# LuckyLYM/Zebra

Hardware: AMD Instinct MI355X
Metric: temporal edges/sec embedded (k=20, 2-layer) (higher is better)
Workload: dtype f64+f32

## Files before the change

### zebra_amd/csrc/aggregate.hip

```cpp
#include "common.hpp"
#include "embed_out_body.hpp"
#include "fc1_tile.hpp"

using namespace zt;
using namespace zt::dense;

namespace {

constexpr int MAX_MT = 5;
constexpr int MAX_MT_BIG = 16;
constexpr int MAX_MT_BIG_WIDE = 8;

#ifdef ZT_AGG_STAMP
__device__ unsigned long long g_agg[8];
#define AGG_STAMP(i) do { if (threadIdx.x == 0) { const long long t__ = clock64(); atomicAdd(&g_agg[i], (unsigned long long)(t__ - t_prev__)); t_prev__ = t__; } } while (0)
#else
#define AGG_STAMP(i) do { } while (0)
#endif

template <bool TAB, int MMT = MAX_MT, int NW = NTW>
__global__ __launch_bounds__(AGG_THREADS) void k_fc1_agg(FcAggArgs a, int rq, int mt_count, int lda)
{
    extern __shared__ __attribute__((aligned(16))) char smem[];
    const float *__restrict__ memory = a.memory, *__restrict__ efeat = a.efeat, *__restrict__ overlay = a.overlay;
// ... 232 lines not shown
        g_nb[tid] = nb; g_ei[tid] = ei; g_dt[tid] = d; wn[tid] = wv;
    }
    const int cc = tid & 127;
    const float wc = cc < T ? time_w[cc] : 0.f;
    const int col0 = wave * 16 + r16;
    const float bias0 = col0 < D ? b1[col0] : 0.f, bias1 = (wave < 3 && col0 + 64 < D) ? b1[col0 + 64] : 0.f;
    __syncthreads();
    AGG_STAMP(0);

    f32x4 acc[5][2];
#pragma unroll
    for (int a = 0; a < 5; ++a) {
        const int nb4[4] = {g_nb[a * 16 + g4 * 4 + 0], g_nb[a * 16 + g4 * 4 + 1], g_nb[a * 16 + g4 * 4 + 2], g_nb[a * 16 + g4 * 4 + 3]};
#pragma unroll
        for (int j = 0; j < 4; ++j) {
            const float *pr = P + (size_t)nb4[j] * DP + col0;
            acc[a][0][j] = pr[0];
            acc[a][1][j] = pr[wave < 3 ? 64 : 0];
        }
    }
    if (tid < ROWS) {
        const int q = tid / KK;
        float my_sum = 0.f;
#pragma unroll
        for (int j = 0; j < KK; ++j) my_sum += wn[q * KK + j];
        wnn[tid] = (my_sum == 0.f) ? 0.f : wn[tid] / my_sum;
        if (tid < rows && tid - q * KK == 0) S[(size_t)m * N + q0 + q] = (my_sum == 0.f) ? 0.f : 1.f;
    }
    AGG_STAMP(1);
    if (F == 1) {
        if (tid < ROWS) A[(size_t)tid * lda] = ef1;
    } else if (F > 0) {
        constexpr int GU = 8;
        const bool vecF = (F & 3) == 0 && ((size_t)efeat & 15) == 0;
        if (vecF) {
            const int F4 = F >> 2;
            const unsigned mF4 = fastdiv_magic((unsigned)F4);
            for (int f0 = tid; f0 < ROWS * F4; f0 += AGG_THREADS * GU) {
                f32x4 v[GU];
#pragma unroll
                for (int u = 0; u < GU; ++u) {
                    const int f = f0 + u * AGG_THREADS;
                    const int g = fastdiv(f, mF4), c = f - g * F4;
                    v[u] = (f < ROWS * F4 && g < rows) ? *reinterpret_cast<const f32x4 *>(efeat + (size_t)g_ei[g] * F + 4 * c)
                                                      : f32x4{0.f, 0.f, 0.f, 0.f};
                }
#pragma unroll
                for (int u = 0; u < GU; ++u) {
                    const int f = f0 + u * AGG_THREADS;
                    const int g = fastdiv(f, mF4), c = f - g * F4;
                    if (f < ROWS * F4) *reinterpret_cast<f32x4 *>(A + (size_t)g * lda + 4 * c) = v[u];
                }
            }
        } else {
            const unsigned mF = fastdiv_magic((unsigned)F);
            for (int f0 = tid; f0 < ROWS * F; f0 += AGG_THREADS * GU) {
                float v[GU];
#pragma unroll
                for (int u = 0; u < GU; ++u) {
                    const int f = f0 + u * AGG_THREADS;
                    const int g = fastdiv(f, mF), c = f - g * F;
                    v[u] = (f < ROWS * F && g < rows) ? efeat[(size_t)g_ei[g] * F + c] : 0.f;
                }
#pragma unroll
                for (int u = 0; u < GU; ++u) {
                    const int f = f0 + u * AGG_THREADS;
                    const int g = fastdiv(f, mF), c = f - g * F;
                    if (f < ROWS * F) A[(size_t)g * lda + c] = v[u];
                }
            }
        }
    }
    {
        const int g0 = (tid >> 7) * 40;
        const bool is_cos = cc < T;
        if (is_cos || F + cc < K1p) {
            float *dst = A + (size_t)g0 * lda + F + cc;
            float xmax = 0.f;
#pragma unroll 2
            for (int i = 0; i < 40; i += 4) {
                const f32x4 d4 = *reinterpret_cast<const f32x4 *>(g_dt + g0 + i);
#pragma unroll
                for (int u = 0; u < 4; ++u) {
                    const float x = d4[u] * wc;
                    xmax = fmaxf(xmax, fabsf(x));
                    dst[(size_t)(i + u) * lda] = time_cosf_fast(x);
                }
            }
            if (!is_cos) {
                for (int i = 0; i < 40; ++i) dst[(size_t)i * lda] = 0.f;
            } else if (!(xmax < 4.0e6f)) {
                for (int i = 0; i < 40; ++i) dst[(size_t)i * lda] = time_cosf(g_dt[g0 + i] * wc);
            }
        }
    }
    AGG_STAMP(2);
    AGG_STAMP(3);
    __syncthreads();
    AGG_STAMP(4);

    {
        const float *bp = W1p + (size_t)col0 * K1p + 4 * g4;
        const int K4 = (F + T + 3) & ~3, nchunk = K4 >> 4, nrem = (K4 & 15) >> 2;
        if (wave < 3) d100_mfma<2>(A, lda, bp, K1p, nchunk, nrem, r16, g4, acc);
        else          d100_mfma<1>(A, lda, bp, K1p, nchunk, nrem, r16, g4, acc);
    }
    AGG_STAMP(5);
    __syncthreads();

    float *Hs = A;
    {
        float *hp = Hs + (size_t)(g4 * 4) * LDH + col0;
#pragma unroll
        for (int a = 0; a < 5; ++a) {
            const f32x4 w4 = *reinterpret_cast<const f32x4 *>(wnn + a * 16 + g4 * 4);
#pragma unroll
            for (int j = 0; j < 4; ++j) {
                float v = acc[a][0][j] + bias0;
                v = v > 0.f ? v : 0.f;
                hp[(size_t)(a * 16 + j) * LDH] = v * w4[j];
            }
        }
        if (wave < 3) {
#pragma unroll
            for (int a = 0; a < 5; ++a) {
                const f32x4 w4 = *reinterpret_cast<const f32x4 *>(wnn + a * 16 + g4 * 4);
#pragma unroll
                for (int j = 0; j < 4; ++j) {
                    float v1 = acc[a][1][j] + bias1;
                    v1 = v1 > 0.f ? v1 : 0.f;
                    hp[(size_t)(a * 16 + j) * LDH + 64] = v1 * w4[j];
                }
            }
        }
    }
    __syncthreads();
    AGG_STAMP(6);
    if (cc < D) {
        for (int q = tid >> 7; q < nq; q += 2) {
            const float *hq = Hs + (size_t)(q * KK) * LDH + cc;
            float s = 0.f;
#pragma unroll
            for (int j = 0; j < KK; ++j) s += hq[(size_t)j * LDH];
            H[((size_t)m * N + q0 + q) * D + cc] = s;
        }
    }
    AGG_STAMP(7);
}

#ifdef ZT_DIAG
__device__ unsigned long long g_regclk[4 * 1024];
#endif
constexpr int REG_NS = 26;
constexpr int REG_NB = 7;
constexpr int REG_FRAG_GROUPS = (REG_NB * REG_NS + 3) / 4;

__global__ void k_pack_reg_frag(const float *__restrict__ W1t, int K2p, float *__restrict__ image)
{
    const int i = blockIdx.x * blockDim.x + threadIdx.x;
    if (i >= REG_FRAG_GROUPS * 64 * 4) return;
    const int e = i & 3, lane = (i >> 2) & 63, G = i >> 8;
    const int q = 4 * G + e, b = q / REG_NS, st = q % REG_NS;
    image[i] = q < REG_NB * REG_NS ? W1t[(16 * b + (lane & 15)) * K2p + 4 * st + (lane >> 4)] : 0.f;
}

template <int KK, int DBG = 0>
__global__ __launch_bounds__(AGG_THREADS, 1) void k_fc1_agg_reg(
    const float *__restrict__ P, const float *__restrict__ efeat, const float *__restrict__ time_w, long long num_nodes,
    long long num_edges, int F, long long N, int M, const int *__restrict__ nbr, const int *__restrict__ eix,
    const float *__restrict__ dt, const float *__restrict__ w, const float *__restrict__ Wfrag,
    const float *__restrict__ b1, float *__restrict__ H, float *__restrict__ S, int *status,
    const int *gate_word, int gate_target, int *gate_latch)
{
    constexpr int D = 100, T = 100, DP = 112, ROWS = 80, RQ = ROWS / KK;
    static_assert(KK % 4 == 0 && ROWS % KK == 0, "groups of 4 rows must not straddle query rows");
    __shared__ int s_nb[AGG_WAVES][ROWS];
    __shared__ __attribute__((aligned(16))) float s_dt[AGG_WAVES][ROWS];
    __shared__ __attribute__((aligned(16))) float s_w[AGG_WAVES][ROWS];
    __shared__ float s_sum[AGG_WAVES][4];
    __shared__ __attribute__((aligned(16))) float s_ef[AGG_WAVES][ROWS * 4];
    const int lane = threadIdx.x & 63, wave = threadIdx.x >> 6;
    const int r16 = lane & 15, g4 = lane >> 4;
    int *nb_s = s_nb[wave];
    float *dt_s = s_dt[wave], *w_s = s_w[wave], *sum_s = s_sum[wave], *ef_s = s_ef[wave];
#ifdef ZT_DIAG
    const unsigned long long wall_in = DBG ? __builtin_amdgcn_s_memrealtime() : 0ull;
#endif

    float Breg[REG_NB][REG_NS];
    {
        const f32x4 *Wf = reinterpret_cast<const f32x4 *>(Wfrag) + lane;
        static_assert(REG_FRAG_GROUPS % 2 == 0, "two batches");
        constexpr int HB = REG_FRAG_GROUPS / 2;
#pragma unroll
        for (int half = 0; half < 2; ++half) {
            f32x4 v[HB];
#pragma unroll
            for (int i = 0; i < HB; ++i) v[i] = Wf[(half * HB + i) * 64];
            __builtin_amdgcn_sched_barrier(0);
#pragma unroll
            for (int i = 0; i < HB; ++i)
#pragma unroll
                for (int e = 0; e < 4; ++e) {
                    const int q = 4 * (half * HB + i) + e;
                    if (q < REG_NB * REG_NS) asm volatile("v_accvgpr_write_b32 %0, %1" : "=a"(Breg[q / REG_NS][q % REG_NS]) : "v"(v[i][e]));
                }
            __builtin_amdgcn_sched_barrier(0);
        }
    }
    float freq[REG_NS];
#pragma unroll
    for (int st = 0; st < REG_NS; ++st) {
        const int kc = 4 * st + g4 - F;
        freq[st] = (kc >= 0 && kc < T) ? time_w[kc] : 0.f;
    }
    float bias[REG_NB];
#pragma unroll
    for (int b = 0; b < REG_NB; ++b) bias[b] = (16 * b + r16) < D ? b1[16 * b + r16] : 0.f;

#ifdef ZT_DIAG
    const unsigned long long clk0 = DBG ? __builtin_amdgcn_s_memtime() : 0ull, wall0 = DBG ? __builtin_amdgcn_s_memrealtime() : 0ull;
#endif
    const long long tpm = (N + RQ - 1) / RQ;
    const long long n_tiles = tpm * M;
    const long long stride = (long long)gridDim.x * AGG_WAVES;
    long long tile = (long long)blockIdx.x * AGG_WAVES + wave;

    int pf_nb[2] = {0, 0}, pf_ei[2] = {0, 0};
    float pf_dt[2] = {0.f, 0.f}, pf_w[2] = {0.f, 0.f};
    auto fetch = [&](long long t) {
        const long long m = t / tpm, q0 = (t - m * tpm) * RQ;
        const int rows = (int)((N - q0) < RQ ? (N - q0) : RQ) * KK;
        const size_t mb = ((size_t)m * N + q0) * KK;
#pragma unroll
        for (int h = 0; h < 2; ++h) {
            const int row = h * 64 + lane;
            const bool in = row < rows && (h == 0 || lane < ROWS - 64);
            pf_nb[h] = in ? nbr[mb + row] : 0;
            pf_ei[h] = in ? eix[mb + row] : 0;
            pf_dt[h] = in ? dt[mb + row] : 0.f;
            pf_w[h] = in ? w[mb + row] : 0.f;
        }
    };
    float pf_ef[2][4] = {{0.f, 0.f, 0.f, 0.f}, {0.f, 0.f, 0.f, 0.f}};
    auto fetch_ef = [&]() {
#pragma unroll
        for (int h = 0; h < 2; ++h) {
            const int ei = pf_ei[h];
            const bool ok = ei >= 0 && ei < num_edges && (h == 0 || lane < ROWS - 64);
#pragma unroll
            for (int c = 0; c < 4; ++c) pf_ef[h][c] = (ok && c < F) ? efeat[(size_t)ei * F + c] : 0.f;
        }
    };
    member_gate_enter(gate_word, gate_target, status, gate_latch);
    if (tile < n_tiles) { fetch(tile); fetch_ef(); }

#pragma nounroll
    for (; tile < n_tiles; tile += stride) {
        const long long m = tile / tpm, q0 = (tile - m * tpm) * RQ;
        const int nq = (int)((N - q0) < RQ ? (N - q0) : RQ);
#pragma unroll
        for (int h = 0; h < 2; ++h) {
            const int row = h * 64 + lane;
            if (h == 0 || lane < ROWS - 64) {
                int nb = pf_nb[h], ei = pf_ei[h];
                if (nb < 0 || nb >= num_nodes || ei < 0 || ei >= num_edges) { atomicExch(status, ZT_ERR_RANGE); nb = 0; ei = 0; }
                nb_s[row] = nb; dt_s[row] = pf_dt[h]; w_s[row] = pf_w[h];
                *reinterpret_cast<f32x4 *>(ef_s + 4 * row) = f32x4{pf_ef[h][0], pf_ef[h][1], pf_ef[h][2], pf_ef[h][3]};
            }
        }
        wave_sync();
        if (lane < RQ) {
            f32x4 wv[KK / 4];
#pragma unroll
            for (int j = 0; j < KK / 4; ++j) wv[j] = *reinterpret_cast<const f32x4 *>(w_s + lane * KK + 4 * j);
            float sm = 0.f;
#pragma unroll
            for (int j = 0; j < KK; ++j) sm += wv[j / 4][j % 4];
            sum_s[lane] = sm;
            if (lane < nq) S[(size_t)m * N + q0 + lane] = (sm == 0.f) ? 0.f : 1.f;
        }
        wave_sync();
#pragma unroll
        for (int h = 0; h < 2; ++h) {
            const int row = h * 64 + lane;
            if (h == 0 || lane < ROWS - 64) {
                const float qs = sum_s[row / KK];
                w_s[row] = (qs == 0.f) ? 0.f : pf_w[h] / qs;
            }
        }
        wave_sync();
        const bool has_next = tile + stride < n_tiles;
        if (has_next) fetch(tile + stride);

        float Hloc[RQ][REG_NB];
#pragma unroll
        for (int q = 0; q < RQ; ++q)
#pragma unroll
            for (int b = 0; b < REG_NB; ++b) Hloc[q][b] = 0.f;

        f32x4 acc[REG_NB];
        float accv[REG_NB][4], Pv[2][REG_NB][4], wn_cur[4], wn_prv[4];
        auto load_P = [&](int x) {
            const int4 nb4 = *reinterpret_cast<const int4 *>(nb_s + x * 16 + 4 * g4);
            const float *p0 = P + (size_t)nb4.x * DP + r16, *p1 = P + (size_t)nb4.y * DP + r16,
                        *p2 = P + (size_t)nb4.z * DP + r16, *p3 = P + (size_t)nb4.w * DP + r16;
#pragma unroll
            for (int b = 0; b < REG_NB; ++b) {
                Pv[x & 1][b][0] = p0[16 * b]; Pv[x & 1][b][1] = p1[16 * b]; Pv[x & 1][b][2] = p2[16 * b]; Pv[x & 1][b][3] = p3[16 * b];
            }
        };
        if (!(DBG & 4)) { load_P(0); load_P(1); }
#pragma unroll
        for (int a = 0; a <= 5; ++a) {
            float dta = 0.f, A_next[2] = {0.f, 0.f};
            if (a > 0) {
#pragma unroll
                for (int b = 0; b < REG_NB; ++b)
#pragma unroll
                    for (int j = 0; j < 4; ++j) accv[b][j] = acc[b][j];
#pragma unroll
                for (int j = 0; j < 4; ++j) wn_prv[j] = wn_cur[j];
            }
            if (a < 5) {
                dta = dt_s[a * 16 + r16];
                const float ef = ef_s[4 * (a * 16 + r16) + (g4 & 3)];
                const f32x4 w4 = *reinterpret_cast<const f32x4 *>(w_s + a * 16 + 4 * g4);
#pragma unroll
                for (int j = 0; j < 4; ++j) wn_cur[j] = w4[j];
#pragma unroll
                for (int b = 0; b < REG_NB; ++b) acc[b] = f32x4{bias[b], bias[b], bias[b], bias[b]};
                A_next[0] = (DBG & 1) ? dta * freq[0] : time_cosf_rev(dta * freq[0]);
                A_next[1] = (DBG & 1) ? dta * freq[1] : time_cosf_rev(dta * freq[1]);
                if (g4 < F) A_next[0] = ef;
                if (a == 2 && has_next) fetch_ef();
            }
            __builtin_amdgcn_sched_barrier(0);
            const int ap = a > 0 ? a - 1 : 0;
            const int q_lo = (16 * ap) / KK, q_hi = (16 * ap + 15) / KK;
#pragma unroll
            for (int st0 = 0; st0 < REG_NS; st0 += 2) {
                if (a == 5 && st0 >= REG_NB) break;
                const float A_cur[2] = {A_next[0], A_next[1]};
                if (a < 5) {
#pragma unroll
                    for (int u = 0; u < 2; ++u)
                        if (st0 + 2 + u < REG_NS)
                            A_next[u] = (DBG & 1) ? dta * freq[st0 + 2 + u] : time_cosf_rev(dta * freq[st0 + 2 + u]);
#pragma unroll
                    for (int u = 0; u < 2; ++u)
#pragma unroll
                        for (int b = 0; b < REG_NB; ++b)
                            acc[b] = __builtin_amdgcn_mfma_f32_16x16x4f32(A_cur[u], Breg[b][st0 + u], acc[b], 0, 0, 0);
                }
#pragma unroll
                for (int u = 0; u < 2; ++u) {
                    const int st = st0 + u;
                    if (!(a > 0 && st < REG_NB)) continue;
                    const int b = st;
                    float part = 0.f;
#pragma unroll
                    for (int j = 0; j < 4; ++j) {
                        float v = accv[b][j] + ((DBG & 2) ? 0.f : Pv[ap & 1][b][j]);
                        v = v > 0.f ? v : 0.f;
                        part += (DBG & 2) ? v : v * wn_prv[j];
                    }
                    if (DBG & 2) {
                        Hloc[q_lo][b] += part;
                    } else {
                        const int pi = __float_as_int(part);
                        const auto h = __builtin_amdgcn_permlane32_swap(pi, pi, false, false);
                        const auto lo = __builtin_amdgcn_permlane16_swap(h[0], h[0], false, false);
                        const auto hi = __builtin_amdgcn_permlane16_swap(h[1], h[1], false, false);
                        const float pg[4] = {__int_as_float(lo[0]), __int_as_float(lo[1]), __int_as_float(hi[0]), __int_as_float(hi[1])};
#pragma unroll
                        for (int g = 0; g < 4; ++g) {
                            const int q = (16 * ap + 4 * g) / KK;
                            if (q < RQ) Hloc[q][b] += pg[g];
                        }
                    }
                    asm volatile("" : "+v"(Hloc[q_lo][b]));
                    if (q_hi != q_lo && q_hi < RQ) asm volatile("" : "+v"(Hloc[q_hi][b]));
                }
                if (a >= 1 && a <= 3 && st0 == REG_NB + 1 && !(DBG & 4)) load_P(a + 1);
                __builtin_amdgcn_sched_barrier(0);
            }
        }
#pragma unroll
        for (int q = 0; q < RQ; ++q) {
            if (g4 == (q & 3) && q < nq) {
                float *hrow = H + ((size_t)m * N + q0 + q) * D;
#pragma unroll
                for (int b = 0; b < REG_NB; ++b)
                    if (16 * b + r16 < D) hrow[16 * b + r16] = Hloc[q][b];
            }
        }
        wave_sync();
    }
#ifdef ZT_DIAG
    if (DBG && lane == 0 && blockIdx.x * AGG_WAVES + wave < 1024) {
        unsigned long long *o = g_regclk + 4 * (blockIdx.x * AGG_WAVES + wave);
        o[0] = __builtin_amdgcn_s_memtime() - clk0; o[1] = wall0; o[2] = __builtin_amdgcn_s_memrealtime();
        o[3] = wall_in;
    }
#endif
}


constexpr int EO3_NT = 7, EO3_KC = 7, EO3_DP = 112, EO3_LDY = 116;
constexpr int EO3_FRAG = EO3_NT * EO3_KC * 256;

__device__ __forceinline__ void eo3_fill(float *Wl, const float *__restrict__ Wp, int tid)
{
    constexpr int PER = (EO3_NT * EO3_KC * 64 + 255) / 256;
    f32x4 v[PER];
#pragma unroll
    for (int q = 0; q < PER; ++q) {
        const int idx = tid + q * 256, frag = idx >> 6, ln = idx & 63;
        const int b = frag / EO3_KC, c = frag - b * EO3_KC;
        v[q] = idx < EO3_NT * EO3_KC * 64
                   ? *reinterpret_cast<const f32x4 *>(Wp + (size_t)(16 * b + (ln & 15)) * EO3_DP + 16 * c + 4 * (ln >> 4))
                   : f32x4{0.f, 0.f, 0.f, 0.f};
    }
#pragma unroll
    for (int q = 0; q < PER; ++q) {
        const int idx = tid + q * 256;
        if (idx < EO3_NT * EO3_KC * 64) reinterpret_cast<f32x4 *>(Wl)[idx] = v[q];
    }
}

template <int HG>
__global__ __launch_bounds__(AGG_THREADS, 1) void k_embed_out3(
    const float *__restrict__ memory, long long num_nodes, const int *__restrict__ nodes, long long N, int D, int M,
    const float *__restrict__ H, const float *__restrict__ S, const float *__restrict__ fc2_p,
    const float *__restrict__ fc2_b, const float *__restrict__ fc1s_p, const float *__restrict__ fc1s_b,
    const float *__restrict__ fc2s_p, const float *__restrict__ fc2s_b, float *__restrict__ out, int *status, int n_src)
{
    extern __shared__ __attribute__((aligned(16))) char smem[];
    float *W0 = reinterpret_cast<float *>(smem);
    const int tid = threadIdx.x, lane = tid & 63, wave = tid >> 6, r16 = lane & 15, g4 = lane >> 4;
    const int OW = D * (M + 1);
    const long long tiles = (N + 15) / 16;
    const f32x4 zero4 = {0.f, 0.f, 0.f, 0.f};
    bool cin[EO3_KC];
#pragma unroll
    for (int c = 0; c < EO3_KC; ++c) cin[c] = 16 * c + 4 * g4 < D;
    const f32x4 *Wf0 = reinterpret_cast<const f32x4 *>(W0) + lane;

    if ((int)blockIdx.x < n_src) {
        float *W1 = W0 + EO3_FRAG;
        float *Y = W1 + EO3_FRAG + wave * 16 * EO3_LDY;
        eo3_fill(W0, fc1s_p, tid);
        eo3_fill(W1, fc2s_p, tid);
        float b1v[EO3_NT], b2v[EO3_NT];
#pragma unroll
        for (int b = 0; b < EO3_NT; ++b) {
            b1v[b] = 16 * b + r16 < D ? fc1s_b[16 * b + r16] : 0.f;
            b2v[b] = 16 * b + r16 < D ? fc2s_b[16 * b + r16] : 0.f;
        }
        const f32x4 *Wf1 = reinterpret_cast<const f32x4 *>(W1) + lane;
        const long long stride = (long long)n_src * AGG_WAVES;
        long long t = (long long)blockIdx.x * AGG_WAVES + wave;
        auto node_of = [&](long long tt) -> int { return (tt < tiles && tt * 16 + r16 < N) ? nodes[tt * 16 + r16] : -1; };
        auto rows_of = [&](int nd, f32x4 (&a)[EO3_KC]) {
            const bool ok = nd >= 0 && nd < num_nodes;
#pragma unroll
            for (int c = 0; c < EO3_KC; ++c)
                a[c] = (ok && cin[c]) ? *reinterpret_cast<const f32x4 *>(memory + (size_t)nd * D + 16 * c + 4 * g4) : zero4;
        };
        int nd_cur = node_of(t), nd_nxt = node_of(t + stride);
        f32x4 a[EO3_KC], an[EO3_KC];
        if (t < tiles) rows_of(nd_cur, a);
        __syncthreads();
        for (; t < tiles; t += stride) {
            const long long r0 = t * 16;
            if (r0 + r16 < N && (nd_cur < 0 || nd_cur >= num_nodes)) atomicExch(status, ZT_ERR_RANGE);
            rows_of(nd_nxt, an);
            nd_cur = nd_nxt;
            nd_nxt = node_of(t + 2 * stride);
            f32x4 acc1[EO3_NT];
#pragma unroll
            for (int b = 0; b < EO3_NT; ++b) acc1[b] = zero4;
#pragma unroll
            for (int c = 0; c < EO3_KC; ++c) {
                f32x4 w[EO3_NT];
#pragma unroll
                for (int b = 0; b < EO3_NT; ++b) w[b] = Wf0[(b * EO3_KC + c) * 64];
#pragma unroll
                for (int j = 0; j < 4; ++j)
#pragma unroll
                    for (int b = 0; b < EO3_NT; ++b) acc1[b] = __builtin_amdgcn_mfma_f32_16x16x4f32(a[c][j], w[b][j], acc1[b], 0, 0, 0);
            }
#pragma unroll
            for (int b = 0; b < EO3_NT; ++b)
#pragma unroll
                for (int j = 0; j < 4; ++j) {
                    const float v = acc1[b][j] + b1v[b];
                    Y[(4 * g4 + j) * EO3_LDY + 16 * b + r16] = (16 * b + r16 < D && v > 0.f) ? v : 0.f;
                }
            wave_sync();
            f32x4 acc[EO3_NT];
#pragma unroll
            for (int b = 0; b < EO3_NT; ++b) acc[b] = zero4;
#pragma unroll
            for (int c = 0; c < EO3_KC; ++c) {
                const f32x4 y = *reinterpret_cast<const f32x4 *>(Y + r16 * EO3_LDY + 16 * c + 4 * g4);
                f32x4 w[EO3_NT];
#pragma unroll
                for (int b = 0; b < EO3_NT; ++b) w[b] = Wf1[(b * EO3_KC + c) * 64];
#pragma unroll
                for (int j = 0; j < 4; ++j)
#pragma unroll
                    for (int b = 0; b < EO3_NT; ++b) acc[b] = __builtin_amdgcn_mfma_f32_16x16x4f32(y[j], w[b][j], acc[b], 0, 0, 0);
            }
#pragma unroll
            for (int b = 0; b < EO3_NT; ++b) {
// ... 128 lines not shown
    size_t lds2;
    size_t off_w1p, off_H, off_S, off_fc2t, off_fc1st, off_fc2st, off_w1t, off_wm, off_wl, off_wfrag, total;
    int hg;
};

bool tile_shape(int Kp, int Dp, int k, int T, int *lda_out, int *mt_out, int *rq_out, size_t *lds_out, int max_mt = MAX_MT)
{
    const int lda = Kp + 4;
    int mt = max_mt;
    while (mt > 1 && ((size_t)mt * 16 * lda * 4 + (size_t)mt * 16 * 16) > (size_t)AGG_LDS_BUDGET) --mt;
    int rq = (mt * 16) / k;
    if (rq < 1) {
        mt = (k + 15) / 16;
        rq = 1;
        if (mt > max_mt || ((size_t)mt * 16 * lda * 4 + (size_t)mt * 16 * 16) > (size_t)AGG_LDS_BUDGET) return false;
    }
    mt = (rq * k + 15) / 16;
    if ((size_t)mt * 16 * (Dp + 1) * 4 > (size_t)mt * 16 * lda * 4) return false;
    *lda_out = lda; *mt_out = mt; *rq_out = rq;
    *lds_out = (size_t)mt * 16 * lda * 4 + (size_t)mt * 16 * 16 + (size_t)T * 4;
    return true;
}

bool split_fits(int D, int F, int T, int k) { return k <= ZT_MAX_K_WIDE && fc1_agg_split_rows(D, F, T) > 0; }

bool make_plan(int64_t N, int D, int F, int T, int M, int k, EmbedPlan &p)
{
    if (!width_supported(D)) return false;
    const int K1 = D + F + T;
    p.Dp = round_up(D, 16);
    p.K1p = round_up(K1, 16);
    const bool big = k > MAX_MT * 16;
    const int max_mt = big ? (p.Dp > 16 * NTW * AGG_WAVES ? MAX_MT_BIG_WIDE : MAX_MT_BIG) : MAX_MT;
    const bool full_ok = tile_shape(p.K1p, p.Dp, k, T, &p.lda, &p.mt, &p.rq, &p.lds, max_mt);
    if (!full_ok) { p.mt = 0; p.rq = 1; p.lda = p.K1p + 4; p.lds = 0; }
    p.K2p = round_up(F + T, 16);
    p.mt2 = 0;
    if (!(full_ok || big) || !tile_shape(p.K2p, p.Dp, k, T, &p.lda2, &p.mt2, &p.rq2, &p.lds2, max_mt)) p.mt2 = 0;
    if (p.mt == 0 && p.mt2 == 0 && !split_fits(D, F, T, k)) return false;
    size_t o = 0;
    auto take = [&](size_t bytes) { size_t r = o; o += (bytes + 255) & ~(size_t)255; return r; };
    p.off_w1p = take((size_t)p.Dp * p.K1p * 4);
    p.off_fc2t = take((size_t)p.Dp * p.Dp * 4);
    p.off_fc1st = take((size_t)p.Dp * p.Dp * 4);
    p.off_fc2st = take((size_t)p.Dp * p.Dp * 4);
    p.off_w1t = take((size_t)p.Dp * p.K2p * 4);
    p.off_wm = take((size_t)p.Dp * p.Dp * 4);
    p.hg = fc1_agg_wide_supported(D, F, T, k) ? k / 4 : 1;
    p.off_wl = take(p.hg > 1 ? fc1_agg_wide_weight_bytes() : 0);
    p.off_wfrag = take((size_t)REG_FRAG_GROUPS * 64 * 4 * 4);
    p.off_H = take((size_t)M * N * D * 4 * p.hg);
    p.off_S = take((size_t)M * N * 4);
    p.total = o;
    return true;
}

KernelPlan plan_kernels(int64_t N, int D, int F, int T, int M, int k, bool have_table, bool training, int agg_choice,
                        int out_choice, EmbedPlan &p)
{
    KernelPlan kp{AggKernel::unsupported, OutForm::tiled, Refusal::shape, 0, 0, 0, 0, 1};
    static_assert(16 * NTW * AGG_WAVES == 128 && 16 * NTW_WIDE * AGG_WAVES == MAX_D, "the N-tiles cover D <= 128 / D <= 256");
    if (!make_plan(N, D, F, T, M, k, p)) return kp;
    const bool big = k > MAX_MT * 16;
    const bool tab = have_table && !training && p.mt2 > 0;
    const bool special = tab && agg_choice != ZT_AGG_GENERIC;
    if (training ? (big || p.mt == 0) : (!tab && p.mt == 0)) {
        if (!split_fits(D, F, T, k)) { kp.refusal = Refusal::no_split; return kp; }
        kp.agg = AggKernel::split;
    } else if (special && p.hg > 1) {
        kp.agg = AggKernel::wide;
    } else if (special && D == 100 && T == 100 && F <= 4 && (k == 20 || k == 40) && p.K2p == 112) {
        kp.agg = AggKernel::reg;
    } else if (special && D == 100 && T == 100 && p.mt2 == 5 && (k == 10 || k == 20 || k == 40)) {
        kp.agg = AggKernel::d100;
    } else if (tab) {
        kp.agg = big ? AggKernel::tiled_table_big : AggKernel::tiled_table;
    } else {
        kp.agg = big ? AggKernel::tiled_full_big : AggKernel::tiled_full;
    }
    if (kp.agg == AggKernel::d100 || kp.agg == AggKernel::tiled_table || kp.agg == AggKernel::tiled_table_big) {
        kp.lds = p.lds2; kp.rq = p.rq2; kp.mt = p.mt2; kp.lda = p.lda2;
    } else if (kp.agg == AggKernel::tiled_full || kp.agg == AggKernel::tiled_full_big) {
        kp.lds = p.lds; kp.rq = p.rq; kp.mt = p.mt; kp.lda = p.lda;
    }
    kp.hg = kp.agg == AggKernel::wide ? p.hg : 1;
    if (kp.hg != 1 && kp.hg != 5 && kp.hg != 10) { kp.agg = AggKernel::unsupported; kp.refusal = Refusal::groups; return kp; }
    kp.refusal = Refusal::none;
    if (D % 4 == 0 && (p.Dp == 112 || p.Dp == 128) && (out_choice == ZT_OUT_LATENCY || (out_choice == 0 && N <= 1024)))
        kp.out = OutForm::latency;
    else if (D % 4 == 0 && p.Dp == EO3_DP && (out_choice == ZT_OUT_PERSIST || (out_choice == 0 && N >= 8192)))
        kp.out = OutForm::persist;
    return kp;
}

}

KernelPlan zt::embed_kernel_plan(int64_t N, int D, int F, int T, int M, int k, bool have_table, bool training, int agg_choice,
                                 int out_choice)
{
    EmbedPlan p;
    return plan_kernels(N, D, F, T, M, k, have_table, training, agg_choice, out_choice, p);
}

#ifdef ZT_AGG_STAMP
extern "C" int zt_debug_agg(unsigned long long *host, int reset)
{
    ZT_HIP(hipDeviceSynchronize());
    ZT_HIP(hipMemcpyFromSymbol(host, HIP_SYMBOL(g_agg), sizeof(unsigned long long) * 8));
    if (reset) { unsigned long long z[8] = {0}; ZT_HIP(hipMemcpyToSymbol(HIP_SYMBOL(g_agg), z, sizeof(z))); }
    return ZT_OK;
}
#endif

#ifdef ZT_DIAG
extern "C" int zt_debug_regclk(unsigned long long *host)
{
    ZT_HIP(hipDeviceSynchronize());
    ZT_HIP(hipMemcpyFromSymbol(host, HIP_SYMBOL(g_regclk), sizeof(unsigned long long) * 4 * 1024));
    return ZT_OK;
}
#endif

extern "C" int64_t zt_embed_workspace_bytes(int64_t N, int32_t D, int32_t F, int32_t T, int32_t M, int32_t k)
{
    EmbedPlan p;
    if (N < 0 || D <= 0 || F < 0 || T < 0 || M <= 0 || k <= 0) return -1;
    if (!make_plan(N > 0 ? N : 1, D, F, T, M, k, p)) return -1;
    return (int64_t)p.total;
}

extern "C" int32_t zt_agg_train_supported(int64_t N, int32_t D, int32_t F, int32_t T, int32_t M, int32_t k)
{
    if (N < 0 || D <= 0 || F < 0 || T < 0 || M <= 0 || k <= 0) return 0;
    EmbedPlan p;
    const KernelPlan kp = plan_kernels(N > 0 ? N : 1, D, F, T, M, k, false, true, 0, 0, p);
    return kp.refusal == Refusal::none && agg_backward_supported(D, F, T, k) ? 1 : 0;
}

static void embed_prepare(const zt_embed_weights *wt, int D, int F, int T, const EmbedPlan &p, char *ws, hipStream_t s)
{
    const int K1 = D + F + T;
    auto pad = [&](const float *W, int ld, int c0, int cols, size_t off, int cols_p) {
        k_pad_matrix<<<(p.Dp * cols_p + 255) / 256, 256, 0, s>>>(W, ld, c0, D, cols, reinterpret_cast<float *>(ws + off), p.Dp, cols_p);
    };
    pad(wt->fc1_w, K1, 0, K1, p.off_w1p, p.K1p);
    pad(wt->fc2_w, D, 0, D, p.off_fc2t, p.Dp);
    pad(wt->fc1s_w, D, 0, D, p.off_fc1st, p.Dp);
    pad(wt->fc2s_w, D, 0, D, p.off_fc2st, p.Dp);
    pad(wt->fc1_w, K1, D, F + T, p.off_w1t, p.K2p);
    pad(wt->fc1_w, K1, 0, D, p.off_wm, p.Dp);
    if (p.hg > 1) fc1_agg_wide_pack(wt->fc1_w, wt->time_w, wt->fc1_b, reinterpret_cast<float *>(ws + p.off_wl), s);
    if (p.K2p == 112 && p.Dp == 112)
        k_pack_reg_frag<<<(REG_FRAG_GROUPS * 64 * 4 + 255) / 256, 256, 0, s>>>(reinterpret_cast<const float *>(ws + p.off_w1t), p.K2p,
                                                                          reinterpret_cast<float *>(ws + p.off_wfrag));
}

const float *zt::embed_wm_ptr(void *embed_ws, int64_t N, int32_t D, int32_t F, int32_t T, int32_t M, int32_t k)
{
    EmbedPlan p;
    if (!embed_ws || !make_plan(N > 0 ? N : 1, D, F, T, M, k, p)) return nullptr;
    return reinterpret_cast<const float *>(reinterpret_cast<char *>(embed_ws) + p.off_wm);
}

extern "C" int64_t zt_project_table_bytes(int64_t num_nodes, int32_t D)
{
    if (num_nodes <= 0 || D <= 0) return -1;
    return (int64_t)num_nodes * round_up(D, 16) * 4;
}

extern "C" int zt_project_memory(const float *memory_dev, int64_t num_nodes, int32_t D, int32_t F, int32_t T,
                                 const zt_embed_weights *wt, int32_t weights_ready, const int32_t *rows_dev,
                                 const int32_t *count_dev, int64_t max_rows, float *table_dev, void *workspace_dev,
                                 int64_t ws_N, int32_t ws_M, int32_t ws_k, void *stream)
{
    if (!memory_dev || !wt || !table_dev || !workspace_dev || num_nodes <= 0 || D <= 0 || F < 0 || T < 0 || max_rows < 0) {
        set_error("zt_project_memory: bad argument");
        return ZT_ERR_ARG;
    }
    EmbedPlan p;
    if (!make_plan(ws_N > 0 ? ws_N : 1, D, F, T, ws_M, ws_k, p)) {
        set_error("zt_project_memory: unsupported shape");
        return ZT_ERR_UNSUPPORTED;
    }
    hipStream_t s = (hipStream_t)stream;
    char *ws = reinterpret_cast<char *>(workspace_dev);
    if (!weights_ready) embed_prepare(wt, D, F, T, p, ws, s);
    const long long n = rows_dev ? max_rows : num_nodes;
    if (n == 0) return ZT_OK;
    const size_t lds = (size_t)OUT_ROWS * (p.Dp + 4) * 4 + OUT_ROWS * 4;
    const auto project = p.Dp > 16 * NTW * AGG_WAVES ? k_project_rows<NTW_WIDE> : k_project_rows<NTW>;
    project<<<(unsigned)((n + OUT_ROWS - 1) / OUT_ROWS), AGG_THREADS, lds, s>>>(
        memory_dev, num_nodes, D, reinterpret_cast<const float *>(ws + p.off_wm), rows_dev, count_dev, n, table_dev);
    ZT_LAUNCH_CHECK();
    return ZT_OK;
}

static int embed_impl(const float *memory_dev, const float *efeat_dev, int64_t num_nodes, int64_t num_edges,
                      int32_t D, int32_t F, int32_t T, const int32_t *nodes_dev, int64_t N, int32_t M, int32_t k,
                      const int32_t *nbr_dev, const int32_t *eix_dev, const float *dt_dev, const float *w_dev,
                      const zt_embed_weights *wt, float *out_dev, void *workspace_dev, int32_t *status_dev,
                      const float *proj_table_dev, int32_t weights_ready, void *stream, hipEvent_t mid_wait,
                      zt::embed_out_deferred *defer = nullptr, const zt::member_gate *gate = nullptr)
{
    if (defer) defer->valid = false;
    if (!memory_dev || !efeat_dev || !wt || !status_dev || N < 0 || D <= 0 || F < 0 || T < 0 || M <= 0 || k <= 0) {
        set_error("zt_embed: bad argument");
        return ZT_ERR_ARG;
    }
    if (N == 0) return ZT_OK;
    if (!nodes_dev || !nbr_dev || !eix_dev || !dt_dev || !w_dev || !out_dev || !workspace_dev) {
        set_error("zt_embed: NULL buffer");
        return ZT_ERR_ARG;
    }
    EmbedPlan p;
    const KernelPlan kp = plan_kernels(N, D, F, T, M, k, proj_table_dev != nullptr, false, kernel_choice(ZT_CHOICE_AGGREGATE),
                                       kernel_choice(ZT_CHOICE_EMBED_OUT), p);
    if (kp.refusal == Refusal::shape) {
        set_error("zt_embed: D=%d F=%d T=%d k=%d outside the supported shapes (D <= 128, or a multiple of 4 up to %d; one query "
                  "row of k neighbours must fit the %d KB LDS tile)", D, F, T, k, MAX_D, AGG_LDS_BUDGET / 1024);
        return ZT_ERR_UNSUPPORTED;
    }
    hipStream_t s = (hipStream_t)stream;
    char *ws = reinterpret_cast<char *>(workspace_dev);
    float *H = reinterpret_cast<float *>(ws + p.off_H);
    float *S = reinterpret_cast<float *>(ws + p.off_S);
    if (!weights_ready) {
        ZT_PROF_BEGIN(s, P_EMBED_PREP);
        embed_prepare(wt, D, F, T, p, ws, s);
        ZT_PROF_END(s, P_EMBED_PREP);
    }
    if (kp.refusal == Refusal::no_split) {
        set_error("zt_embed: k=%d needs the projected table (a query row's [memory | ef | time] tile does not fit %d KB of LDS, "
                  "nor does a chunk of it)", k, AGG_LDS_BUDGET / 1024);
        return ZT_ERR_UNSUPPORTED;
    }
    if (kp.refusal == Refusal::groups) { set_error("zt_embed: %d partial-sum groups per row", kp.hg); return ZT_ERR_UNSUPPORTED; }
    const bool waits_inside = kp.agg == AggKernel::wide || kp.agg == AggKernel::reg;
    if (gate != nullptr && gate->word != nullptr && !waits_inside) {
        const int rc = zt::member_gate_launch(*gate, status_dev, s);
        if (rc != ZT_OK) return rc;
    }
    const dim3 tile_grid((unsigned)(kp.rq > 0 ? (N + kp.rq - 1) / kp.rq : 0), (unsigned)M);
    const bool wide = p.Dp > 16 * NTW * AGG_WAVES;
    FcAggArgs fa{};
    fa.memory = memory_dev; fa.efeat = efeat_dev; fa.time_w = wt->time_w;
    fa.num_nodes = num_nodes; fa.num_edges = num_edges; fa.N = N;
    fa.D = D; fa.F = F; fa.T = T; fa.M = M; fa.k = k; fa.ldm = D;
    fa.nbr = nbr_dev; fa.eix = eix_dev; fa.dt = dt_dev; fa.w = w_dev;
    fa.W1p = reinterpret_cast<const float *>(ws + p.off_w1p); fa.K1p = p.K1p; fa.b1 = wt->fc1_b;
    fa.H = H; fa.S = S; fa.status = status_dev;
    fa.set_dropout(0.f, 0ull);
    auto tiled = [&](decltype(&k_fc1_agg<false>) fn, bool table) {
        FcAggArgs ta = fa;
        if (table) { ta.memory = proj_table_dev; ta.ldm = p.Dp; ta.W1p = reinterpret_cast<const float *>(ws + p.off_w1t); ta.K1p = p.K2p; }
        ZT_HIP(set_dynamic_lds(reinterpret_cast<const void *>(fn), kp.lds));
        fn<<<tile_grid, AGG_THREADS, kp.lds, s>>>(ta, kp.rq, kp.mt, kp.lda);
        return ZT_OK;
    };
    auto reg = [&](decltype(&k_fc1_agg_reg<20>) fn) {
        const long long rq = 80 / k, tiles = ((N + rq - 1) / rq) * M;
        long long wgs = (tiles + AGG_WAVES - 1) / AGG_WAVES;
        const int cus = stream_cu_count(s);
        if (wgs > cus) wgs = cus;
        fn<<<(unsigned)wgs, AGG_THREADS, 0, s>>>(proj_table_dev, efeat_dev, wt->time_w, num_nodes, num_edges, F, N, M, nbr_dev, eix_dev,
                                                 dt_dev, w_dev, reinterpret_cast<const float *>(ws + p.off_wfrag), wt->fc1_b, H, S,
                                                 status_dev, gate ? gate->word : nullptr, gate ? gate->target : 0,
                                                 gate ? gate->latch : nullptr);
        return ZT_OK;
    };
    ZT_PROF_BEGIN(s, P_FC1_AGG);
    int rc = ZT_OK;
    switch (kp.agg) {
    case AggKernel::wide:
        rc = fc1_agg_wide_launch(proj_table_dev, efeat_dev, wt->time_w, num_nodes, num_edges, N, M, k, nbr_dev, eix_dev, dt_dev,
                                 w_dev, reinterpret_cast<const float *>(ws + p.off_wl), wt->fc1_b, H, S, status_dev,
                                 stream_cu_count(s), s, gate);
        break;
    case AggKernel::reg:
#ifdef ZT_DIAG
        {
            static const int dbg = getenv("ZT_AGG_DBG") ? atoi(getenv("ZT_AGG_DBG")) : 0;
            if (k == 20 && dispatch<1, 2, 6, 7, 8>(dbg, [&](auto DB) { return reg(k_fc1_agg_reg<20, DB>); }) == ZT_OK) break;
        }
#endif
        rc = dispatch<20, 40>(k, [&](auto KK) { return reg(k_fc1_agg_reg<KK>); });
        break;
    case AggKernel::d100:
        rc = dispatch<10, 20, 40>(k, [&](auto KK) {
            ZT_HIP(set_dynamic_lds(reinterpret_cast<const void *>(k_fc1_agg_d100<KK>), kp.lds));
            k_fc1_agg_d100<KK><<<tile_grid, AGG_THREADS, kp.lds, s>>>(proj_table_dev, efeat_dev, wt->time_w, num_nodes, num_edges, F, N,
                                                                     kp.lda, nbr_dev, eix_dev, dt_dev, w_dev,
                                                                     reinterpret_cast<const float *>(ws + p.off_w1t), p.K2p, wt->fc1_b,
                                                                     H, S, status_dev);
            return ZT_OK;
        });
        break;
    case AggKernel::tiled_table: rc = tiled(wide ? k_fc1_agg<true, MAX_MT, NTW_WIDE> : k_fc1_agg<true>, true); break;
    case AggKernel::tiled_table_big: rc = tiled(wide ? k_fc1_agg<true, MAX_MT_BIG_WIDE, NTW_WIDE> : k_fc1_agg<true, MAX_MT_BIG>, true); break;
    case AggKernel::tiled_full: rc = tiled(wide ? k_fc1_agg<false, MAX_MT, NTW_WIDE> : k_fc1_agg<false>, false); break;
    case AggKernel::tiled_full_big: rc = tiled(wide ? k_fc1_agg<false, MAX_MT_BIG_WIDE, NTW_WIDE> : k_fc1_agg<false, MAX_MT_BIG>, false); break;
    case AggKernel::split: rc = fc1_agg_split_launch(fa, s); break;
    case AggKernel::unsupported: break;
    }
    if (rc != ZT_OK) return rc;
    ZT_PROF_END(s, P_FC1_AGG);
    if (mid_wait != nullptr) ZT_HIP(hipStreamWaitEvent(s, mid_wait, 0));
    const EmbedOutArgs E{memory_dev, num_nodes, nodes_dev, N, D, M, H, S,
                         reinterpret_cast<const float *>(ws + p.off_fc2t), wt->fc2_b,
                         reinterpret_cast<const float *>(ws + p.off_fc1st), wt->fc1s_b,
                         reinterpret_cast<const float *>(ws + p.off_fc2st), wt->fc2s_b, out_dev, status_dev};
    const long long tiles = (N + 15) / 16;
    const zt::embed_out_deferred od{true, E, kp.hg, kp.out, kp.out == OutForm::latency ? (int)(tiles < 256 ? tiles : 256) : 0, nullptr};
    if (defer != nullptr && kp.out != OutForm::persist) {
        int *latch = defer->latch;
        *defer = od;
        defer->latch = latch;
        ZT_LAUNCH_CHECK();
        return ZT_OK;
    }
    ZT_PROF_BEGIN(s, P_EMBED_OUT);
    rc = zt::embed_out_launch(od, s);
    if (rc != ZT_OK) return rc;
    ZT_PROF_END(s, P_EMBED_OUT);
    ZT_LAUNCH_CHECK();
    return ZT_OK;
}

extern "C" int zt_embed(const float *memory_dev, const float *efeat_dev, int64_t num_nodes, int64_t num_edges,
                        int32_t D, int32_t F, int32_t T, const int32_t *nodes_dev, int64_t N, int32_t M, int32_t k,
                        const int32_t *nbr_dev, const int32_t *eix_dev, const float *dt_dev, const float *w_dev,
                        const zt_embed_weights *wt, float *out_dev, void *workspace_dev, int32_t *status_dev,
                        const float *proj_table_dev, int32_t weights_ready, void *stream)
{
    return embed_impl(memory_dev, efeat_dev, num_nodes, num_edges, D, F, T, nodes_dev, N, M, k, nbr_dev, eix_dev, dt_dev, w_dev,
                      wt, out_dev, workspace_dev, status_dev, proj_table_dev, weights_ready, stream, nullptr);
}

int zt::embed_out_launch(const zt::embed_out_deferred &d, void *stream)
{
    hipStream_t s = (hipStream_t)stream;
    const EmbedOutArgs &E = d.args;
    const int Dp = round_up(E.D, 16);
    int rc;
    if (d.form == OutForm::latency) {
        const dim3 grid2((unsigned)d.gx, (unsigned)(E.M + 1), (unsigned)(Dp / 16));
        rc = dispatch<7, 8>(Dp / 16, [&](auto NTV) {
            return dispatch<1, 5, 10>(d.hg, [&](auto HGV) { k_embed_out2<NTV, HGV><<<grid2, 64, 0, s>>>(E); return ZT_OK; });
        });
    } else if (d.form == OutForm::persist) {
        const long long tiles = (E.N + 15) / 16;
        long long wgs = zt::stream_cu_count(s);
        const long long want = (tiles * (E.M + 2) + AGG_WAVES - 1) / AGG_WAVES;
        if (wgs > want) wgs = want;
        if (wgs < 2) wgs = 2;
        int n_src = (int)((2 * wgs + (E.M + 2) / 2) / (E.M + 2));
        if (n_src < 1) n_src = 1;
        if (n_src > wgs - 1) n_src = (int)wgs - 1;
        const size_t lds3 = (size_t)(2 * EO3_FRAG + AGG_WAVES * 16 * EO3_LDY) * 4;
        rc = dispatch<1, 5, 10>(d.hg, [&](auto HGV) {
            ZT_HIP(set_dynamic_lds(reinterpret_cast<const void *>(k_embed_out3<HGV>), lds3));
            k_embed_out3<HGV><<<(unsigned)wgs, AGG_THREADS, lds3, s>>>(E.memory, E.num_nodes, E.nodes, E.N, E.D, E.M, E.H, E.S, E.fc2_p,
                                                                      E.fc2_b, E.fc1s_p, E.fc1s_b, E.fc2s_p, E.fc2s_b, E.out, E.status,
                                                                      n_src);
            return ZT_OK;
        });
    } else {
        const size_t lds2 = (size_t)2 * OUT_ROWS * (Dp + 4) * 4 + OUT_ROWS * 4;
        const dim3 grid((unsigned)((E.N + OUT_ROWS - 1) / OUT_ROWS), (unsigned)(E.M + 1));
        if (Dp > 16 * NTW * AGG_WAVES) {
            rc = dispatch<1>(d.hg, [&](auto HGV) {
                ZT_HIP(set_dynamic_lds(reinterpret_cast<const void *>(k_embed_out<HGV, NTW_WIDE>), lds2));
                k_embed_out<HGV, NTW_WIDE><<<grid, AGG_THREADS, lds2, s>>>(E);
                return ZT_OK;
            });
        } else {
            rc = dispatch<1, 5, 10>(d.hg, [&](auto HGV) { k_embed_out<HGV><<<grid, AGG_THREADS, lds2, s>>>(E); return ZT_OK; });
        }
    }
    if (rc == ZT_ERR_UNSUPPORTED) set_error("zt_embed: %d partial-sum groups per row", d.hg);
    if (rc != ZT_OK) return rc;
    ZT_LAUNCH_CHECK();
    return ZT_OK;
}

int zt::embed_ex(const float *memory_dev, const float *efeat_dev, int64_t num_nodes, int64_t num_edges,
                 int32_t D, int32_t F, int32_t T, const int32_t *nodes_dev, int64_t N, int32_t M, int32_t k,
                 const int32_t *nbr_dev, const int32_t *eix_dev, const float *dt_dev, const float *w_dev,
                 const zt_embed_weights *wt, float *out_dev, void *workspace_dev, int32_t *status_dev,
                 const float *proj_table_dev, int32_t weights_ready, void *stream, hipEvent_t mid_wait,
                 zt::embed_out_deferred *defer, const zt::member_gate *gate)
{
    return embed_impl(memory_dev, efeat_dev, num_nodes, num_edges, D, F, T, nodes_dev, N, M, k, nbr_dev, eix_dev, dt_dev, w_dev,
                      wt, out_dev, workspace_dev, status_dev, proj_table_dev, weights_ready, stream, mid_wait, defer, gate);
}

namespace {
__global__ void k_member_gate(const int *word, int target, int *status, int *latch)
{
    if (threadIdx.x == 0) (void)member_gate_wait(word, target, status, latch);
}
}

int zt::member_gate_launch(const zt::member_gate &g, int32_t *status_dev, void *stream)
{
    if (g.word == nullptr) return ZT_OK;
    k_member_gate<<<1, 64, 0, (hipStream_t)stream>>>(g.word, g.target, status_dev, g.latch);
    ZT_LAUNCH_CHECK();
    return ZT_OK;
}

extern "C" int zt_agg_train_forward(const float *memory_dev, const float *overlay_dev, const int32_t *row_map_dev,
                                    const float *efeat_dev, int64_t num_nodes, int64_t num_edges, int32_t D, int32_t F,
                                    int32_t T, int64_t N, int32_t M, int32_t k, const int32_t *nbr_dev,
                                    const int32_t *eix_dev, const float *dt_dev, const float *w_dev,
                                    const zt_embed_weights *wt, float *H_dev, float *S_dev, void *workspace_dev,
                                    int32_t *status_dev, float drop_p, uint64_t drop_seed, void *stream)
{
    if (!memory_dev || !efeat_dev || !wt || !status_dev || !H_dev || !S_dev || !workspace_dev || N < 0 || D <= 0 || F < 0 ||
        T < 0 || M <= 0 || k <= 0 || (row_map_dev != nullptr && !overlay_dev) || !(drop_p >= 0.f && drop_p < 1.f)) {
        set_error("zt_agg_train_forward: bad argument");
        return ZT_ERR_ARG;
    }
    if (N == 0) return ZT_OK;
    EmbedPlan p;
    const KernelPlan kp = plan_kernels(N, D, F, T, M, k, false, true, 0, 0, p);
    if (kp.refusal == Refusal::shape) {
        set_error("zt_agg_train_forward: unsupported shape");
        return ZT_ERR_UNSUPPORTED;
    }
    if (kp.refusal == Refusal::no_split) {
        set_error("zt_agg_train_forward: D=%d F=%d T=%d k=%d: no 16-row chunk fits %d KB of LDS", D, F, T, k, AGG_LDS_BUDGET / 1024);
        return ZT_ERR_UNSUPPORTED;
    }
    hipStream_t s = (hipStream_t)stream;
    char *ws = reinterpret_cast<char *>(workspace_dev);
    embed_prepare(wt, D, F, T, p, ws, s);
    FcAggArgs fa{};
    fa.memory = memory_dev; fa.efeat = efeat_dev; fa.time_w = wt->time_w;
// ... 17 lines not shown
```

Baseline: 14.19 million.

## Handle last output block with 4x4 MFMA and fold single edge feature as rank-1 term

```diff
diff --git a/zebra_amd/csrc/aggregate.hip b/zebra_amd/csrc/aggregate.hip
--- a/zebra_amd/csrc/aggregate.hip
+++ b/zebra_amd/csrc/aggregate.hip
@@ -408,19 +408,28 @@
 __device__ unsigned long long g_regclk[4 * 1024];
 #endif
 constexpr int REG_NS = 26;
+constexpr int REG_NS_EF1 = 25;
 constexpr int REG_NB = 7;
+#ifndef ZT_AGG_EF1
+#define ZT_AGG_EF1 1
+#endif
 constexpr int REG_FRAG_GROUPS = (REG_NB * REG_NS + 3) / 4;
 
-__global__ void k_pack_reg_frag(const float *__restrict__ W1t, int K2p, float *__restrict__ image)
+__global__ void k_pack_reg_frag(const float *__restrict__ W1t, int K2p, int ef1, float *__restrict__ image)
 {
     const int i = blockIdx.x * blockDim.x + threadIdx.x;
     if (i >= REG_FRAG_GROUPS * 64 * 4) return;
     const int e = i & 3, lane = (i >> 2) & 63, G = i >> 8;
-    const int q = 4 * G + e, b = q / REG_NS, st = q % REG_NS;
-    image[i] = q < REG_NB * REG_NS ? W1t[(16 * b + (lane & 15)) * K2p + 4 * st + (lane >> 4)] : 0.f;
-}
-
-template <int KK, int DBG = 0>
+    const int ns = ef1 ? REG_NS_EF1 : REG_NS, q = 4 * G + e;
+    const int b = q < REG_NB * ns ? q / ns : q - REG_NB * ns, st = q % ns;
+    const int row = b < REG_NB - 1 ? 16 * b + (lane & 15) : 96 + (lane & 3);
+    float v = 0.f;
+    if (q < REG_NB * ns) v = W1t[row * K2p + (ef1 ? 1 : 0) + 4 * st + (lane >> 4)];
+    else if (ef1 && b < REG_NB) v = W1t[row * K2p];
+    image[i] = v;
+}
+
+template <int KK, int DBG = 0, bool EF1 = false>
 __global__ __launch_bounds__(AGG_THREADS, 1) void k_fc1_agg_reg(
     const float *__restrict__ P, const float *__restrict__ efeat, const float *__restrict__ time_w, long long num_nodes,
     long long num_edges, int F, long long N, int M, const int *__restrict__ nbr, const int *__restrict__ eix,
@@ -429,7 +438,11 @@
     const int *gate_word, int gate_target, int *gate_latch)
 {
     constexpr int D = 100, T = 100, DP = 112, ROWS = 80, RQ = ROWS / KK;
+    constexpr int NS = EF1 ? REG_NS_EF1 : REG_NS, TAIL = REG_NB - 1;
+    constexpr int TB1 = 8, TB2 = 16, TBN = NS - TB2;
+    static_assert(TB1 % 2 == 0 && TB2 % 2 == 0 && TB2 < NS, "a batch ends with a round of two steps");
     static_assert(KK % 4 == 0 && ROWS % KK == 0, "groups of 4 rows must not straddle query rows");
+    static_assert(REG_NB * NS + (EF1 ? REG_NB : 0) <= 4 * REG_FRAG_GROUPS, "the image holds a lane's values");
     __shared__ int s_nb[AGG_WAVES][ROWS];
     __shared__ __attribute__((aligned(16))) float s_dt[AGG_WAVES][ROWS];
     __shared__ __attribute__((aligned(16))) float s_w[AGG_WAVES][ROWS];
@@ -437,13 +450,17 @@
     __shared__ __attribute__((aligned(16))) float s_ef[AGG_WAVES][ROWS * 4];
     const int lane = threadIdx.x & 63, wave = threadIdx.x >> 6;
     const int r16 = lane & 15, g4 = lane >> 4;
+    const int rg4 = 4 * (r16 >> 2);
     int *nb_s = s_nb[wave];
     float *dt_s = s_dt[wave], *w_s = s_w[wave], *sum_s = s_sum[wave], *ef_s = s_ef[wave];
 #ifdef ZT_DIAG
     const unsigned long long wall_in = DBG ? __builtin_amdgcn_s_memrealtime() : 0ull;
 #endif
 
-    float Breg[REG_NB][REG_NS];
+    float Breg[REG_NB][NS];
+    float w0[REG_NB];
+#pragma unroll
+    for (int b = 0; b < REG_NB; ++b) w0[b] = 0.f;
     {
         const f32x4 *Wf = reinterpret_cast<const f32x4 *>(Wfrag) + lane;
         static_assert(REG_FRAG_GROUPS % 2 == 0, "two batches");
@@ -459,20 +476,21 @@
 #pragma unroll
                 for (int e = 0; e < 4; ++e) {
                     const int q = 4 * (half * HB + i) + e;
-                    if (q < REG_NB * REG_NS) asm volatile("v_accvgpr_write_b32 %0, %1" : "=a"(Breg[q / REG_NS][q % REG_NS]) : "v"(v[i][e]));
+                    if (q < REG_NB * NS) asm volatile("v_accvgpr_write_b32 %0, %1" : "=a"(Breg[q / NS][q % NS]) : "v"(v[i][e]));
+                    else if (EF1 && q < REG_NB * NS + REG_NB) w0[q - REG_NB * NS] = v[i][e];
                 }
             __builtin_amdgcn_sched_barrier(0);
         }
     }
-    float freq[REG_NS];
-#pragma unroll
-    for (int st = 0; st < REG_NS; ++st) {
-        const int kc = 4 * st + g4 - F;
+    float freq[NS];
+#pragma unroll
+    for (int st = 0; st < NS; ++st) {
+        const int kc = 4 * st + g4 - (EF1 ? 0 : F);
         freq[st] = (kc >= 0 && kc < T) ? time_w[kc] : 0.f;
     }
     float bias[REG_NB];
 #pragma unroll
-    for (int b = 0; b < REG_NB; ++b) bias[b] = (16 * b + r16) < D ? b1[16 * b + r16] : 0.f;
+    for (int b = 0; b < REG_NB; ++b) bias[b] = b1[b < TAIL ? 16 * b + r16 : 96 + (r16 & 3)];
 
 #ifdef ZT_DIAG
     const unsigned long long clk0 = DBG ? __builtin_amdgcn_s_memtime() : 0ull, wall0 = DBG ? __builtin_amdgcn_s_memrealtime() : 0ull;
@@ -555,28 +573,41 @@
 #pragma unroll
             for (int b = 0; b < REG_NB; ++b) Hloc[q][b] = 0.f;
 
-        f32x4 acc[REG_NB];
+        f32x4 acc[TAIL], accT[2];
+        float At[TBN > TB1 ? TBN : TB1];
         float accv[REG_NB][4], Pv[2][REG_NB][4], wn_cur[4], wn_prv[4];
         auto load_P = [&](int x) {
             const int4 nb4 = *reinterpret_cast<const int4 *>(nb_s + x * 16 + 4 * g4);
             const float *p0 = P + (size_t)nb4.x * DP + r16, *p1 = P + (size_t)nb4.y * DP + r16,
                         *p2 = P + (size_t)nb4.z * DP + r16, *p3 = P + (size_t)nb4.w * DP + r16;
 #pragma unroll
-            for (int b = 0; b < REG_NB; ++b) {
+            for (int b = 0; b < TAIL; ++b) {
                 Pv[x & 1][b][0] = p0[16 * b]; Pv[x & 1][b][1] = p1[16 * b]; Pv[x & 1][b][2] = p2[16 * b]; Pv[x & 1][b][3] = p3[16 * b];
             }
+            Pv[x & 1][TAIL][0] = P[(size_t)nb_s[x * 16 + rg4 + g4] * DP + 96 + (r16 & 3)];
         };
         if (!(DBG & 4)) { load_P(0); load_P(1); }
 #pragma unroll
         for (int a = 0; a <= 5; ++a) {
             float dta = 0.f, A_next[2] = {0.f, 0.f};
+            float wt_prv[4] = {0.f, 0.f, 0.f, 0.f}, ef_prv[4] = {0.f, 0.f, 0.f, 0.f}, eft_prv = 0.f;
             if (a > 0) {
 #pragma unroll
-                for (int b = 0; b < REG_NB; ++b)
+                for (int b = 0; b < TAIL; ++b)
 #pragma unroll
                     for (int j = 0; j < 4; ++j) accv[b][j] = acc[b][j];
 #pragma unroll
+                for (int j = 0; j < 4; ++j) accv[TAIL][j] = accT[0][j] + accT[1][j];
+#pragma unroll
                 for (int j = 0; j < 4; ++j) wn_prv[j] = wn_cur[j];
+                const f32x4 wt4 = *reinterpret_cast<const f32x4 *>(w_s + (a - 1) * 16 + rg4);
+#pragma unroll
+                for (int j = 0; j < 4; ++j) wt_prv[j] = wt4[j];
+                if (EF1) {
+#pragma unroll
+                    for (int j = 0; j < 4; ++j) ef_prv[j] = ef_s[4 * ((a - 1) * 16 + 4 * g4 + j)];
+                    eft_prv = ef_s[4 * ((a - 1) * 16 + rg4 + g4)];
+                }
             }
             if (a < 5) {
                 dta = dt_s[a * 16 + r16];
@@ -585,29 +616,41 @@
 #pragma unroll
                 for (int j = 0; j < 4; ++j) wn_cur[j] = w4[j];
 #pragma unroll
-                for (int b = 0; b < REG_NB; ++b) acc[b] = f32x4{bias[b], bias[b], bias[b], bias[b]};
+                for (int b = 0; b < TAIL; ++b) acc[b] = f32x4{bias[b], bias[b], bias[b], bias[b]};
+                accT[0] = accT[1] = f32x4{0.f, 0.f, 0.f, 0.f};
                 A_next[0] = (DBG & 1) ? dta * freq[0] : time_cosf_rev(dta * freq[0]);
                 A_next[1] = (DBG & 1) ? dta * freq[1] : time_cosf_rev(dta * freq[1]);
-                if (g4 < F) A_next[0] = ef;
+                if (!EF1 && g4 < F) A_next[0] = ef;
                 if (a == 2 && has_next) fetch_ef();
             }
             __builtin_amdgcn_sched_barrier(0);
             const int ap = a > 0 ? a - 1 : 0;
             const int q_lo = (16 * ap) / KK, q_hi = (16 * ap + 15) / KK;
 #pragma unroll
-            for (int st0 = 0; st0 < REG_NS; st0 += 2) {
+            for (int st0 = 0; st0 < NS; st0 += 2) {
                 if (a == 5 && st0 >= REG_NB) break;
                 const float A_cur[2] = {A_next[0], A_next[1]};
                 if (a < 5) {
 #pragma unroll
                     for (int u = 0; u < 2; ++u)
-                        if (st0 + 2 + u < REG_NS)
+                        if (st0 + 2 + u < NS)
                             A_next[u] = (DBG & 1) ? dta * freq[st0 + 2 + u] : time_cosf_rev(dta * freq[st0 + 2 + u]);
-#pragma unroll
-                    for (int u = 0; u < 2; ++u)
-#pragma unroll
-                        for (int b = 0; b < REG_NB; ++b)
+                    const int tb = st0 < TB1 ? 0 : st0 < TB2 ? TB1 : TB2;
+#pragma unroll
+                    for (int u = 0; u < 2; ++u) {
+                        if (st0 + u >= NS) continue;
+#pragma unroll
+                        for (int b = 0; b < TAIL; ++b)
                             acc[b] = __builtin_amdgcn_mfma_f32_16x16x4f32(A_cur[u], Breg[b][st0 + u], acc[b], 0, 0, 0);
+                        At[st0 + u - tb] = A_cur[u];
+                    }
+                    if (st0 + 2 == TB1 || st0 + 2 == TB2 || st0 + 2 >= NS) {
+                        __builtin_amdgcn_sched_barrier(0);
+#pragma unroll
+                        for (int s = tb; s < NS && s < st0 + 2; ++s)
+                            accT[s & 1] = __builtin_amdgcn_mfma_f32_4x4x1f32(At[s - tb], Breg[TAIL][s], accT[s & 1], 0, 0, 0);
+                        __builtin_amdgcn_sched_barrier(0);
+                    }
                 }
 #pragma unroll
                 for (int u = 0; u < 2; ++u) {
@@ -615,9 +658,37 @@
                     if (!(a > 0 && st < REG_NB)) continue;
                     const int b = st;
                     float part = 0.f;
+                    if (b == TAIL && !(DBG & 2)) {
+                        const auto x01 = __builtin_amdgcn_permlane16_swap(__float_as_int(accv[b][0]), __float_as_int(accv[b][1]), false, false);
+                        const auto x23 = __builtin_amdgcn_permlane16_swap(__float_as_int(accv[b][2]), __float_as_int(accv[b][3]), false, false);
+                        const float s01 = __int_as_float(x01[0]) + __int_as_float(x01[1]);
+                        const float s23 = __int_as_float(x23[0]) + __int_as_float(x23[1]);
+                        const auto xs = __builtin_amdgcn_permlane32_swap(__float_as_int(s01), __float_as_int(s23), false, false);
+                        float v = (__int_as_float(xs[0]) + __int_as_float(xs[1])) + bias[b];
+                        v += Pv[ap & 1][b][0];
+                        if (EF1) v = fmaf(eft_prv, w0[b], v);
+                        v = v > 0.f ? v : 0.f;
+                        const int vi = __float_as_int(v);
+                        const auto h = __builtin_amdgcn_permlane32_swap(vi, vi, false, false);
+                        const auto lo = __builtin_amdgcn_permlane16_swap(h[0], h[0], false, false);
+                        const auto hi = __builtin_amdgcn_permlane16_swap(h[1], h[1], false, false);
+                        const float vr[4] = {__int_as_float(lo[0]), __int_as_float(lo[1]), __int_as_float(hi[0]), __int_as_float(hi[1])};
+#pragma unroll
+                        for (int j = 0; j < 4; ++j) part += vr[j] * wt_prv[j];
+                        const float pg[4] = {part, dpp_f<0x104>(part), dpp_f<0x108>(part), dpp_f<0x10C>(part)};
+#pragma unroll
+                        for (int g = 0; g < 4; ++g) {
+                            const int q = (16 * ap + 4 * g) / KK;
+                            if (q < RQ) Hloc[q][b] += pg[g];
+                        }
+                        asm volatile("" : "+v"(Hloc[q_lo][b]));
+                        if (q_hi != q_lo && q_hi < RQ) asm volatile("" : "+v"(Hloc[q_hi][b]));
+                        continue;
+                    }
 #pragma unroll
                     for (int j = 0; j < 4; ++j) {
                         float v = accv[b][j] + ((DBG & 2) ? 0.f : Pv[ap & 1][b][j]);
+                        if (EF1 && !(DBG & 2)) v = fmaf(ef_prv[j], w0[b], v);
                         v = v > 0.f ? v : 0.f;
                         part += (DBG & 2) ? v : v * wn_prv[j];
                     }
@@ -1052,6 +1123,7 @@
     if (p.hg > 1) fc1_agg_wide_pack(wt->fc1_w, wt->time_w, wt->fc1_b, reinterpret_cast<float *>(ws + p.off_wl), s);
     if (p.K2p == 112 && p.Dp == 112)
         k_pack_reg_frag<<<(REG_FRAG_GROUPS * 64 * 4 + 255) / 256, 256, 0, s>>>(reinterpret_cast<const float *>(ws + p.off_w1t), p.K2p,
+                                                                          ZT_AGG_EF1 && F == 1,
                                                                           reinterpret_cast<float *>(ws + p.off_wfrag));
 }
 
@@ -1180,10 +1252,11 @@
 #ifdef ZT_DIAG
         {
             static const int dbg = getenv("ZT_AGG_DBG") ? atoi(getenv("ZT_AGG_DBG")) : 0;
-            if (k == 20 && dispatch<1, 2, 6, 7, 8>(dbg, [&](auto DB) { return reg(k_fc1_agg_reg<20, DB>); }) == ZT_OK) break;
+            if (k == 20 && dispatch<1, 2, 6, 7, 8>(dbg, [&](auto DB) {
+                    return reg(ZT_AGG_EF1 && F == 1 ? k_fc1_agg_reg<20, DB, true> : k_fc1_agg_reg<20, DB>); }) == ZT_OK) break;
         }
 #endif
-        rc = dispatch<20, 40>(k, [&](auto KK) { return reg(k_fc1_agg_reg<KK>); });
+        rc = dispatch<20, 40>(k, [&](auto KK) { return reg(ZT_AGG_EF1 && F == 1 ? k_fc1_agg_reg<KK, 0, true> : k_fc1_agg_reg<KK>); });
         break;
     case AggKernel::d100:
         rc = dispatch<10, 20, 40>(k, [&](auto KK) {
```

New measurement: 14.14 million. Within noise of the previous version (-0.4%).
